# Adamtaranto/mimeo

Hardware: AMD Instinct MI355X
Metric: Gbp-aligned/sec (mimeo self, 1 Gbp genome, --minIdt 80 --minLen 100 --minCov 3) (higher is better)
Workload: dtype int32

## Files before the change

### mimeo_amd/csrc/device_util.h

```cpp
#pragma once
#include "common.h"

namespace mimeo {

#define MIMEO_AS_GLOBAL __attribute__((address_space(1)))
template <class T> struct gnative { using type = T; };
template <> struct gnative<uint2> { using type = uint32_t __attribute__((ext_vector_type(2))); };
template <> struct gnative<uint4> { using type = uint32_t __attribute__((ext_vector_type(4))); };
template <class T>
struct gptr {
    using N = typename gnative<T>::type;
    static_assert(sizeof(N) == sizeof(T), "the native twin has the layout of T");
    const MIMEO_AS_GLOBAL N *p;
    gptr() = default;
    __device__ __forceinline__ gptr(const T *q) : p((const MIMEO_AS_GLOBAL N *)q) {}
    __device__ __forceinline__ explicit gptr(const MIMEO_AS_GLOBAL N *q) : p(q) {}
    template <class I> __device__ __forceinline__ T operator[](I i) const { const N v = p[i]; return __builtin_bit_cast(T, v); }
    template <class I> __device__ __forceinline__ gptr operator+(I i) const { return gptr(p + i); }
    __device__ __forceinline__ explicit operator bool() const { return p != nullptr; }
    template <class U> __device__ __forceinline__ gptr<U> as() const { return gptr<U>((const MIMEO_AS_GLOBAL typename gnative<U>::type *)p); }
};
struct GStrandView {
    gptr<uint4> pw;
    gptr<uint32_t> svt;
// ... 37 lines not shown
    r.nm = (uint32_t)((((uint64_t)c.z << 32) | a.z) >> b);
    r.sv = (uint32_t)((((uint64_t)c.w << 32) | a.w) >> b);
    return r;
}
__device__ __forceinline__ Win64 win64(const GStrandView &v, int32_t s) {
    const int32_t w = s >> 5;
    const uint32_t b = (uint32_t)s & 31u;
    const uint4 a = v.pw[w], c = v.pw[w + 1], e = v.pw[w + 2];
    Win64 r;
    uint64_t l;
    l = ((uint64_t)c.x << 32) | a.x; r.lo = b ? (l >> b) | ((uint64_t)e.x << (64 - b)) : l;
    l = ((uint64_t)c.y << 32) | a.y; r.hi = b ? (l >> b) | ((uint64_t)e.y << (64 - b)) : l;
    l = ((uint64_t)c.z << 32) | a.z; r.nm = b ? (l >> b) | ((uint64_t)e.z << (64 - b)) : l;
    l = ((uint64_t)c.w << 32) | a.w; r.sv = b ? (l >> b) | ((uint64_t)e.w << (64 - b)) : l;
    return r;
}
template <class P>
__device__ __forceinline__ uint32_t get32(const P pl, int32_t s) {
    int32_t w = s >> 5;
    uint32_t b = (uint32_t)s & 31u;
    uint64_t v = (uint64_t)pl[w] | ((uint64_t)pl[w + 1] << 32);
    return (uint32_t)(v >> b);
}
__device__ __forceinline__ uint32_t seedvalid32(const GStrandView &v, int32_t s, uint32_t sv_from_window) {
    return v.svt ? get32(v.svt, s) : sv_from_window;
}
struct Base1 { uint32_t lo, hi, nm; };
__device__ __forceinline__ Base1 base_at(const GStrandView &v, int32_t s) {
    const uint4 a = v.pw[s >> 5];
    const uint32_t b = (uint32_t)s & 31u;
    return Base1{(a.x >> b) & 1u, (a.y >> b) & 1u, (a.z >> b) & 1u};
}

__device__ __forceinline__ int32_t sub_score(uint32_t dl, uint32_t dh, uint32_t cg, uint32_t nn) {
    uint32_t tb = dl ? 0x83858E8Eu : 0xE1E1645Bu;
    uint32_t sh = 24u - (((dh << 1) | cg) << 3);
    int32_t s = ((int32_t)(tb << sh)) >> 24;
    return nn ? -100 : s;
}

__device__ __forceinline__ int32_t pair_score(const GStrandView &T, const GStrandView &Q, int32_t pt, int32_t pq,
                                              bool *is_match) {
    const Base1 a = base_at(T, pt), b = base_at(Q, pq);
    const uint32_t dl = a.lo ^ b.lo, dh = a.hi ^ b.hi, nn = a.nm | b.nm;
    *is_match = !(dl | dh | nn);
    return sub_score(dl, dh, a.lo ^ a.hi, nn);
}

}
```

### mimeo_amd/csrc/k4_device.h

```cpp
#pragma once
#include "device_util.h"

namespace mimeo {

constexpr uint32_t CARE19 = 0x7A997u;
constexpr int EXT_THREADS = 256;
constexpr int LONG_WINDOWS = 8;

struct ExtCounters {
    unsigned long long ncand, nfollow, nlong, nhsp, nmed, nbig, nwalked;
    unsigned long long nfollow8[8], nmed8[8];
    unsigned long long nbigcand;
    unsigned long long long_next, seg_next;
    unsigned long long nwalk_total, nwalk_over;
    unsigned long long dbg[8];
};

struct HeavyPlan {
    const unsigned long long *est;
    uint2 *tile;
    uint32_t *base;
    uint4 *split;
    unsigned int *ctr;
};
struct Cand {
    uint32_t tstart, qstart, len;
    int32_t raw;
    uint32_t unit;
};
constexpr int32_t RAW_SATURATED = 0x7FFFFFFF;

struct ExtQueues {
    ExtCounters *ctr;
    Cand *cand;
    uint64_t *fkey;
    uint32_t *fprev;
    uint2 *medq, *longq;
    uint32_t *medu, *longu;
    uint2 *walkq;
    unsigned long long *nwalk_u;
    unsigned long long *nheavy_u;
    uint32_t *heavy;
    unsigned long long *heavy_est;
    unsigned long long *bigcand;
    unsigned long long *bigacc;
    unsigned long long *unit_hits;
    unsigned long long *tile_hits;
    uint64_t cand_cap, follow_cap, med_cap, long_cap, walk_cap;
    uint32_t ebits, dbits;
};
constexpr uint32_t WALK_SHARP_DONE = 0x80000000u;
__device__ __forceinline__ uint32_t queue_shard() { return blockIdx.x & 7u; }
__device__ __forceinline__ unsigned long long wave_slot(unsigned long long *counter) {
    const uint64_t m = __ballot(true);
    const uint32_t lane = threadIdx.x & 63u, lead = (uint32_t)__builtin_ctzll(m);
    unsigned long long b = 0;
    if (lane == lead) b = atomicAdd(counter, (unsigned long long)__popcll(m));
    b = __shfl(b, (int)lead);
    return b + __popcll(m & ((1ull << lane) - 1ull));
}
__device__ __forceinline__ uint64_t follow_key(const ExtQueues &q, uint32_t unit, int32_t d, uint32_t qlen, uint32_t et) {
    return ((uint64_t)unit << (q.dbits + q.ebits)) | ((uint64_t)(uint32_t)(d + (int32_t)qlen) << q.ebits) | (uint64_t)et;
}
__device__ __forceinline__ uint32_t key_unit(const ExtQueues &q, uint64_t k) { return (uint32_t)(k >> (q.dbits + q.ebits)); }
__device__ __forceinline__ uint32_t key_end(const ExtQueues &q, uint64_t k) { return (uint32_t)(k & ((1ull << q.ebits) - 1ull)); }
__device__ __forceinline__ uint64_t key_unit_diag(const ExtQueues &q, uint64_t k) { return k >> q.ebits; }
__device__ __forceinline__ int32_t key_diag(const ExtQueues &q, uint64_t k, uint32_t qlen) {
    return (int32_t)(uint32_t)((k >> q.ebits) & ((1ull << q.dbits) - 1ull)) - (int32_t)qlen;
}

// ... 87 lines not shown
    int32_t R = w.run, B = w.best, sR = R, sB = B;
    uint32_t BK = 0, sBK = 0, sC = 0;
    bool stopped = w.done, slow = false, brkdone = false;
#pragma unroll
    for (int c = 0; c < NG; c++) {
        const uint32_t e = ent[c];
        const int32_t S = ((int32_t)(e << 22)) >> 22, M = ((int32_t)(e << 12)) >> 22, mn = ((int32_t)(e << 2)) >> 22;
        const bool blk = (nz >> (G * c)) & 1u;
        const bool brk = R + mn + xdrop < B;
        const bool first = (blk || brk) && !stopped;
        sR = first ? R : sR;
        sB = first ? B : sB;
        sBK = first ? BK : sBK;
        sC = first ? (uint32_t)c : sC;
        slow = slow || (first && blk);
        brkdone = brkdone || (first && !blk);
        stopped = stopped || blk || brk;
        const int32_t cand = R + M;
        BK = cand > B ? (e >> 30) + (uint32_t)(G * c + 1) : BK;
        B = max(B, cand);
        R += S;
    }
    if (!stopped) { sR = R; sB = B; sBK = BK; sC = NG; }
    w.run = sR;
    w.best = sB;
    w.bk = sBK ? w.k + sBK : w.bk;
    w.k += (uint32_t)G * sC;
    w.done = w.done || brkdone;
    if (__ballot(slow)) {
        if (slow) walk_window<G>(tab, w, mdl, mdh, mcg, mnn, mH, limit, xdrop, (uint32_t)G * sC);
    }
}

template <int G>
__device__ __forceinline__ uint32_t group_table_entry(uint32_t idx) {
    int32_t p = 0, M = -100000, mn = 100000, posM = 0;
#pragma unroll
    for (int k = 0; k < G; k++) {
        p += sub_score((idx >> k) & 1u, (idx >> (G + k)) & 1u, (idx >> (2 * G + k)) & 1u, 0u);
        if (p > M) { M = p; posM = k; }
        if (p < mn) mn = p;
    }
    return ((uint32_t)p & 0x3FFu) | (((uint32_t)M & 0x3FFu) << 10) | (((uint32_t)mn & 0x3FFu) << 20) | ((uint32_t)posM << 30);
}

__device__ __forceinline__ uint32_t ext32(uint32_t a, uint32_t b, uint32_t c, uint32_t sh) {
    return sh < 32 ? __builtin_amdgcn_alignbit(b, a, sh) : __builtin_amdgcn_alignbit(c, b, sh - 32);
}

struct Frame {
    uint32_t dl[6], dh[6], cg[6], nn[6], st[6], sq[6];
};

struct WinMasks { uint32_t dl, dh, cg, nn, H; };

template <int WIN>
__device__ __forceinline__ WinMasks left_masks(const Frame &F, uint32_t bt, int transitions) {
    constexpr int b = 1 - WIN;
    const uint32_t dllo = __builtin_amdgcn_alignbit(F.dl[b + 1], F.dl[b], bt), dlhi = __builtin_amdgcn_alignbit(F.dl[b + 2], F.dl[b + 1], bt);
    const uint32_t dhlo = __builtin_amdgcn_alignbit(F.dh[b + 1], F.dh[b], bt), dhhi = __builtin_amdgcn_alignbit(F.dh[b + 2], F.dh[b + 1], bt);
    const uint32_t cglo = __builtin_amdgcn_alignbit(F.cg[b + 1], F.cg[b], bt), cghi = __builtin_amdgcn_alignbit(F.cg[b + 2], F.cg[b + 1], bt);
    const uint32_t nnlo = __builtin_amdgcn_alignbit(F.nn[b + 1], F.nn[b], bt), nnhi = __builtin_amdgcn_alignbit(F.nn[b + 2], F.nn[b + 1], bt);
    const uint32_t nlo = dllo | dhlo, nhi = dlhi | dhhi;
    uint32_t ones = 0, twos = 0, tv = 0;
#pragma unroll
    for (int c = 0; c < SEED_LEN; c++) {
// ... 120 lines not shown
            t2 |= __builtin_amdgcn_alignbit(dllo, dlm, c);
        }
        m.H2 = ~(transitions ? (w2 | t2) : o2) & 0xFFFF0000u;
    }
    return m;
}

template <int STEP, bool SLIM>
__device__ __forceinline__ bool hit_needs_walk(const GStrandView &T, const GStrandView &Q, const uint2 h, int xdrop,
                                               int hspthresh, int transitions) {
    Frame F;
    if (SLIM) load_frame_slim(T, Q, h, F);
    else load_frame(T, Q, h, F);
    const uint32_t bt = h.x & 31u;
    const FilterMasks l0 = filter_left<0>(F, bt, transitions), l1 = filter_left<1>(F, bt, transitions);
    const uint32_t rs = bt + SEED_LEN;
    Bound L{0, 0, 0, 0, false}, R{0, 0, 0, 0, false};
    bound_window<STEP, true>(L, l0.dl, l0.dh, l0.cg, xdrop);
    bound_window<STEP, true>(L, l1.dl, l1.dh, l1.cg, xdrop);
    const bool stop64 = L.stop;
    bound_window<16, true, 1>(L, l1.dl2, l1.dh2, l1.cg2, xdrop);
    const uint32_t veto2 = stop64 ? 0u : l1.H2;
    bound_window<STEP, false>(R, ext32(F.dl[2], F.dl[3], F.dl[4], rs), ext32(F.dh[2], F.dh[3], F.dh[4], rs),
                              ext32(F.cg[2], F.cg[3], F.cg[4], rs), xdrop);
    bound_window<STEP, false>(R, ext32(F.dl[3], F.dl[4], F.dl[5], rs), ext32(F.dh[3], F.dh[4], F.dh[5], rs),
                              ext32(F.cg[3], F.cg[4], F.cg[5], rs), xdrop);
    const uint32_t veto = F.nn[0] | F.nn[1] | F.nn[2] | F.nn[3] | F.nn[4] | F.nn[5] | l0.H | l1.H | veto2;
    return !(L.stop && R.stop && L.ub + R.ub < hspthresh && veto == 0);
}

template <int VARIANT>
__device__ __forceinline__ void walk_hit(const uint32_t *__restrict__ tab, const GStrandView &T, const GStrandView &Q,
                                         const uint2 h, int xdrop, int hspthresh, int transitions, bool &q_med,
                                         bool &q_fol, bool &q_cd, uint64_t &r_fk, uint32_t &r_fp, Cand &r_cd) {
    const int32_t et = (int32_t)h.x + SEED_LEN, eq = (int32_t)h.y + SEED_LEN;
    const int32_t d = (int32_t)h.x - (int32_t)h.y;
    const uint32_t bt = h.x & 31u;
    Frame F;
    if (VARIANT == 8) {
        const uint32_t bq = h.y & 31u;
        const int32_t wt = (int32_t)(h.x >> 5) - 2, wq = (int32_t)(h.y >> 5) - 2 - (bq < bt ? 1 : 0);
        const gptr<uint2> t2 = T.pw.as<uint2>(), q2 = Q.pw.as<uint2>();
        uint32_t acc = 0;
#pragma unroll
        for (int k = 0; k < 6; k++) { const uint2 v = t2[wt + k]; acc ^= v.x ^ v.y; }
#pragma unroll
        for (int k = 0; k < 7; k++) { const uint2 v = q2[wq + k]; acc ^= v.x ^ v.y; }
        if (acc == 0x12345678u) q_med = true;
        return;
    }
    if (VARIANT == 3) {
#pragma unroll
        for (int k = 0; k < 6; k++) {
            F.dl[k] = h.x * (k + 1); F.dh[k] = h.y + k; F.cg[k] = h.y * (k + 3); F.nn[k] = 0; F.st[k] = ~0u; F.sq[k] = ~0u;
        }
    } else {
        load_frame(T, Q, h, F);
    }
    if (VARIANT == 2) {
        uint32_t acc = 0;
#pragma unroll
        for (int k = 0; k < 6; k++) acc ^= F.dl[k] ^ F.dh[k] ^ F.cg[k] ^ F.nn[k] ^ F.st[k] ^ F.sq[k];
        if (acc == 0x12345678u) q_med = true;
        return;
    }
    WalkState L{0, 0, 0, 0, false, false, 0};
    const uint32_t maxl = (uint32_t)min(et, eq);
    left_window<0>(tab, F, bt, transitions, L, maxl, xdrop);
    if (!L.done) left_window<1>(tab, F, bt, transitions, L, maxl, xdrop);
    if (!L.done) {
        q_med = true;
    } else if (L.found) {
        q_fol = true;
        r_fk = ((uint64_t)(uint32_t)(d + (int32_t)Q.len) << 32) | (uint32_t)et;
        r_fp = (uint32_t)et - L.found_step;
        if (L.found_step == 1) {
            const bool two_back = seed_hit_at(T, Q, (int32_t)h.x - 2, d, transitions), ahead = seed_hit_at(T, Q, (int32_t)h.x + 1, d, transitions);
            if (two_back && ahead) q_fol = false;
            else if (two_back) r_fp = RUN_END;
        }
    } else {
        WalkState R{0, 0, 0, 0, false, false, 0};
        const uint32_t maxr = min(T.len - (uint32_t)et, Q.len - (uint32_t)eq);
        const uint32_t rs = bt + SEED_LEN;
        walk_window_pred(tab, R, ext32(F.dl[2], F.dl[3], F.dl[4], rs), ext32(F.dh[2], F.dh[3], F.dh[4], rs),
                         ext32(F.cg[2], F.cg[3], F.cg[4], rs), ext32(F.nn[2], F.nn[3], F.nn[4], rs), 0u, maxr, xdrop);
        if (!R.done)
            walk_window_pred(tab, R, ext32(F.dl[3], F.dl[4], F.dl[5], rs), ext32(F.dh[3], F.dh[4], F.dh[5], rs),
                             ext32(F.cg[3], F.cg[4], F.cg[5], rs), ext32(F.nn[3], F.nn[4], F.nn[5], rs), 0u, maxr, xdrop);
        if (!R.done) {
            q_med = true;
        } else if (L.best + R.best >= hspthresh) {
            q_cd = true;
            r_cd = Cand{(uint32_t)et - L.bk, (uint32_t)eq - L.bk, L.bk + R.bk, L.best + R.best, 0u};
        }
    }
}

struct WaveFill { uint32_t n_med, n_fol, n_cd; };

__device__ __forceinline__ uint64_t batch_key(const ExtQueues &q, uint32_t unit, uint64_t staged) {
    return ((uint64_t)unit << (q.dbits + q.ebits)) | ((staged >> 32) << q.ebits) | (staged & 0xFFFFFFFFull);
}

template <bool STAGE_CAND, int CAP = QCAP>
__device__ __forceinline__ void stage_records(const ExtQueues &q, uint32_t unit, uint2 *s_med, uint64_t *s_fk, uint32_t *s_fp,
                                              Cand *s_cd, WaveFill &f, bool q_med, uint2 h, bool q_fol, uint64_t r_fk,
                                              uint32_t r_fp, bool q_cd, Cand r_cd, bool final) {
    const uint32_t lane = threadIdx.x & 63u;
    const uint64_t lt_mask = (1ull << lane) - 1ull;
    uint64_t m = __ballot(q_med);
    if (m || (final && f.n_med)) {
        const uint32_t add = (uint32_t)__popcll(m);
        if (f.n_med + add > (uint32_t)CAP || (final && !m)) {
            __builtin_amdgcn_wave_barrier();
            unsigned long long b = 0;
            if (lane == 0) b = atomicAdd(&q.ctr->nmed8[queue_shard()], (unsigned long long)f.n_med);
            b = __shfl(b, 0);
            for (uint32_t i = lane; i < f.n_med; i += 64)
                if (b + i < q.med_cap) { const size_t at = (size_t)queue_shard() * q.med_cap + b + i; q.medq[at] = s_med[i]; q.medu[at] = unit; }
            f.n_med = 0;
            __builtin_amdgcn_wave_barrier();
        }
        if (q_med) s_med[f.n_med + __popcll(m & lt_mask)] = h;
        f.n_med += add;
        if (final && f.n_med) {
            __builtin_amdgcn_wave_barrier();
            unsigned long long b = 0;
            if (lane == 0) b = atomicAdd(&q.ctr->nmed8[queue_shard()], (unsigned long long)f.n_med);
            b = __shfl(b, 0);
            for (uint32_t i = lane; i < f.n_med; i += 64)
                if (b + i < q.med_cap) { const size_t at = (size_t)queue_shard() * q.med_cap + b + i; q.medq[at] = s_med[i]; q.medu[at] = unit; }
            f.n_med = 0;
        }
    }
    m = __ballot(q_fol);
    if (m || (final && f.n_fol)) {
        const uint32_t add = (uint32_t)__popcll(m);
        if (f.n_fol + add > (uint32_t)CAP || (final && !m)) {
            __builtin_amdgcn_wave_barrier();
            unsigned long long b = 0;
            if (lane == 0) b = atomicAdd(&q.ctr->nfollow8[queue_shard()], (unsigned long long)f.n_fol);
            b = __shfl(b, 0);
            for (uint32_t i = lane; i < f.n_fol; i += 64)
                if (b + i < q.follow_cap) { const size_t at = (size_t)queue_shard() * q.follow_cap + b + i; q.fkey[at] = batch_key(q, unit, s_fk[i]); q.fprev[at] = s_fp[i]; }
            f.n_fol = 0;
            __builtin_amdgcn_wave_barrier();
        }
        if (q_fol) { const uint32_t i = f.n_fol + __popcll(m & lt_mask); s_fk[i] = r_fk; s_fp[i] = r_fp; }
        f.n_fol += add;
        if (final && f.n_fol) {
            __builtin_amdgcn_wave_barrier();
            unsigned long long b = 0;
            if (lane == 0) b = atomicAdd(&q.ctr->nfollow8[queue_shard()], (unsigned long long)f.n_fol);
            b = __shfl(b, 0);
            for (uint32_t i = lane; i < f.n_fol; i += 64)
                if (b + i < q.follow_cap) { const size_t at = (size_t)queue_shard() * q.follow_cap + b + i; q.fkey[at] = batch_key(q, unit, s_fk[i]); q.fprev[at] = s_fp[i]; }
// ... 297 lines not shown
```

### mimeo_amd/csrc/k4_extend.hip

```cpp
#include <algorithm>
#include <cmath>
#include <cstdio>
#include <cstdlib>
#include <cstring>
#include <mutex>
#include <utility>

#include <rocprim/rocprim.hpp>

#include "k4_device.h"

namespace mimeo {

__global__ __launch_bounds__(EXT_THREADS) void k4_extend_generic(const UnitDesc *__restrict__ units, ExtQueues q, int xdrop,
                                                              int hspthresh, int transitions,
                                                              const uint32_t *__restrict__ group_tab) {
    __shared__ uint32_t tab[GROUP_TAB];
    for (int i = threadIdx.x; i < GROUP_TAB; i += EXT_THREADS) tab[i] = group_tab[i];
    __syncthreads();
    uint64_t sh_end[8];
    {
        uint64_t acc = 0;
#pragma unroll
        for (int r = 0; r < 8; r++) { acc += min((uint64_t)q.ctr->nmed8[r], q.med_cap); sh_end[r] = acc; }
// ... 18 lines not shown
        __builtin_amdgcn_wave_barrier();
    };
    auto flush_long = [&]() {
        __builtin_amdgcn_wave_barrier();
        unsigned long long b = 0;
        if (lane == 0) b = atomicAdd(&q.ctr->nlong, (unsigned long long)n_long);
        b = __shfl(b, 0) + lane;
        if (lane < n_long && b < q.long_cap) { q.longq[b] = s_lh[wv][lane]; q.longu[b] = s_lu[wv][lane]; }
        n_long = 0;
        __builtin_amdgcn_wave_barrier();
    };
    auto flush_cd = [&]() {
        __builtin_amdgcn_wave_barrier();
        unsigned long long b = 0;
        if (lane == 0) b = atomicAdd(&q.ctr->ncand, (unsigned long long)n_cd);
        b = __shfl(b, 0) + lane;
        if (lane < n_cd && b < q.cand_cap) q.cand[b] = s_cd[wv][lane];
        n_cd = 0;
        __builtin_amdgcn_wave_barrier();
    };
    const uint64_t stride = (uint64_t)gridDim.x * EXT_THREADS;
    for (uint64_t g0 = (uint64_t)blockIdx.x * EXT_THREADS + wv * 64u; g0 < nhits; g0 += stride) {
        const uint64_t gid = g0 + lane;
        bool o_fol = false, o_long = false, o_cd = false;
        uint64_t r_fk = 0;
        uint32_t r_fp = 0, unit = 0;
        uint2 h = make_uint2(0, 0);
        Cand r_cd{0, 0, 0, 0, 0};
        if (gid < nhits) {
            uint32_t r = 0;
#pragma unroll
            for (int k = 0; k < 7; k++) r += gid >= sh_end[k] ? 1u : 0u;
            const uint64_t at = (uint64_t)r * q.med_cap + (gid - (r ? sh_end[r - 1] : 0));
            h = q.medq[at];
            unit = q.medu[at];
            const GStrandView T = units[unit].T, Q = units[unit].Q;
            const int32_t et = (int32_t)h.x + SEED_LEN, eq = (int32_t)h.y + SEED_LEN;
            const int32_t d = (int32_t)h.x - (int32_t)h.y;
            WalkState L{0, 0, 0, 0, false, false, 0};
            const uint32_t maxl = (uint32_t)min(et, eq);
            bool is_long = false;
            for (int win = 0; !L.done; win++) {
                if (win == LONG_WINDOWS) { is_long = true; break; }
                const int32_t P = et - 32 * (win + 1) - SEED_LEN, Pq = P - d;
                const Win64 tw = win64(T, P), qw = win64(Q, Pq);
                const uint64_t dl64 = tw.lo ^ qw.lo, dh64 = tw.hi ^ qw.hi, nm64 = dl64 | dh64;
                const uint32_t nlo = (uint32_t)nm64, nhi = (uint32_t)(nm64 >> 32);
                const uint32_t tlo = (uint32_t)dl64, thi = (uint32_t)(dl64 >> 32);
                uint32_t ones = 0, twos = 0, tv = 0;
#pragma unroll
                for (int c = 0; c < SEED_LEN; c++) {
                    if (!((CARE19 >> c) & 1u)) continue;
                    const uint32_t v = c ? __builtin_amdgcn_alignbit(nhi, nlo, c) : nlo;
                    twos |= ones & v;
                    ones |= v;
                    tv |= c ? __builtin_amdgcn_alignbit(thi, tlo, c) : tlo;
                }
                const uint32_t bad = transitions ? (twos | tv) : ones;
                const uint32_t H = ~bad & seedvalid32(T, P, (uint32_t)tw.sv) & (uint32_t)qw.sv;
                walk_window(tab, L, __brev((uint32_t)(dl64 >> SEED_LEN)), __brev((uint32_t)(dh64 >> SEED_LEN)),
                            __brev((uint32_t)((tw.lo ^ tw.hi) >> SEED_LEN)), __brev((uint32_t)((tw.nm | qw.nm) >> SEED_LEN)),
                            __brev(H), maxl, xdrop);
            }
            if (!is_long && L.found) {
                o_fol = true;
                r_fk = follow_key(q, unit, d, Q.len, (uint32_t)et);
                r_fp = (uint32_t)et - L.found_step;
            } else {
                WalkState R{0, 0, 0, 0, false, false, 0};
                if (!is_long) {
                    const uint32_t maxr = min(T.len - (uint32_t)et, Q.len - (uint32_t)eq);
                    for (int win = 0; !R.done; win++) {
                        if (win == LONG_WINDOWS) { is_long = true; break; }
                        const int32_t P = et + 32 * win, Pq = P - d;
                        const Win32 tw = win32(T, P), qw = win32(Q, Pq);
                        walk_window(tab, R, tw.lo ^ qw.lo, tw.hi ^ qw.hi, tw.lo ^ tw.hi, tw.nm | qw.nm, 0u, maxr, xdrop);
                    }
                }
                if (is_long) o_long = true;
                else {
                    const int32_t score = L.best + R.best;
                    if (score >= hspthresh) { o_cd = true; r_cd = Cand{(uint32_t)et - L.bk, (uint32_t)eq - L.bk, L.bk + R.bk, score, unit}; }
                }
            }
        }
        uint64_t m = __ballot(o_fol);
        if (m) {
            const uint32_t add = (uint32_t)__popcll(m);
            if (n_fol + add > GCAP) flush_fol();
            if (o_fol) { const uint32_t i = n_fol + (uint32_t)__popcll(m & lt_mask); s_fk[wv][i] = r_fk; s_fp[wv][i] = r_fp; }
            n_fol += add;
        }
        m = __ballot(o_long);
        if (m) {
            const uint32_t add = (uint32_t)__popcll(m);
            if (n_long + add > GCAP) flush_long();
            if (o_long) { const uint32_t i = n_long + (uint32_t)__popcll(m & lt_mask); s_lh[wv][i] = h; s_lu[wv][i] = unit; }
            n_long += add;
        }
        m = __ballot(o_cd);
        if (m) {
            const uint32_t add = (uint32_t)__popcll(m);
            if (n_cd + add > GCAP) flush_cd();
            if (o_cd) s_cd[wv][n_cd + (uint32_t)__popcll(m & lt_mask)] = r_cd;
            n_cd += add;
        }
    }
    if (n_fol) flush_fol();
    if (n_long) flush_long();
    if (n_cd) flush_cd();
}

template <int VARIANT>
__device__ __forceinline__ void extend_hits_body(const GStrandView &T, const GStrandView &Q,
                                                 const uint2 *__restrict__ hits, uint64_t nhits,
                                                 int xdrop, int hspthresh, int transitions,
                                                 const uint32_t *__restrict__ group_tab, const ExtQueues &q, uint32_t unit,
                                                 int skip_diag0, const unsigned long long *__restrict__ nhits_dev) {
    constexpr bool FILTER = VARIANT == 5 || VARIANT == 9;
    constexpr int SCAP = 256;
    uint64_t sh_end[8] = {0, 0, 0, 0, 0, 0, 0, 0};
    const uint64_t shard_cap = nhits;
    if (nhits_dev) {
        uint64_t acc = 0;
#pragma unroll
        for (int r = 0; r < 8; r++) { acc += min((uint64_t)nhits_dev[r], shard_cap); sh_end[r] = acc; }
        nhits = acc;
    }
    __shared__ uint32_t tab[GROUP_TAB];
    __shared__ uint2 s_med[FAST_THREADS / 64][SCAP];
    __shared__ uint64_t s_fk[FAST_THREADS / 64][SCAP];
    __shared__ uint32_t s_fp[FAST_THREADS / 64][SCAP];
    __shared__ Cand s_cd[FAST_THREADS / 64][QCAP];
    __shared__ uint2 s_walk[FILTER ? FAST_THREADS / 64 : 1][QCAP];
    for (int i = threadIdx.x; i < GROUP_TAB; i += FAST_THREADS) tab[i] = group_tab[i];
    __syncthreads();
    const uint32_t lane = threadIdx.x & 63u, wv = threadIdx.x >> 6;
    const uint64_t lt_mask = (1ull << lane) - 1ull;
    WaveFill fill{0, 0, 0};
    uint32_t n_walk = 0, n_walked = 0;

    auto walk_batch = [&](bool active, uint2 h, bool final) {
        bool q_med = false, q_fol = false, q_cd = false;
        uint64_t r_fk = 0;
        uint32_t r_fp = 0;
        Cand r_cd{0, 0, 0, 0, 0};
        if (active) walk_hit<1>(tab, T, Q, h, xdrop, hspthresh, transitions, q_med, q_fol, q_cd, r_fk, r_fp, r_cd);
        stage_records<true, SCAP>(q, unit, s_med[wv], s_fk[wv], s_fp[wv], s_cd[wv], fill, q_med, h, q_fol, r_fk, r_fp, q_cd, r_cd, final);
    };

    const uint64_t stride = (uint64_t)gridDim.x * FAST_THREADS;
    for (uint64_t g0 = (uint64_t)blockIdx.x * FAST_THREADS + wv * 64u; g0 < nhits; g0 += stride) {
        const uint64_t gid = g0 + lane;
        uint2 h = make_uint2(0, 0);
        if (gid < nhits) {
            uint64_t at = gid;
            if (nhits_dev) {
                uint32_t r = 0;
#pragma unroll
                for (int k = 0; k < 7; k++) r += gid >= sh_end[k] ? 1u : 0u;
                at = (uint64_t)r * shard_cap + (gid - (r ? sh_end[r - 1] : 0));
            }
            h = hits[at];
        }
        const bool marked = nhits_dev && (h.x & WALK_SHARP_DONE) != 0;
        if (nhits_dev) h.x &= POS_MASK;
        const bool valid = gid < nhits && !(skip_diag0 && h.x == h.y);
        if (!FILTER) {
            walk_batch(valid, h, false);
        } else {
            bool need = valid && marked;
            if (__ballot(valid && !marked)) {
                if (valid && !marked)
                    need = VARIANT == 9 ? hit_needs_walk<16, true>(T, Q, h, xdrop, hspthresh, transitions)
                                        : hit_needs_walk<16, false>(T, Q, h, xdrop, hspthresh, transitions);
            }
            const uint64_t m = __ballot(need);
            if (m) {
                const uint32_t add = (uint32_t)__popcll(m);
                if (n_walk + add > (uint32_t)QCAP) {
                    __builtin_amdgcn_wave_barrier();
// ... 431 lines not shown
            out_unit[i] = c.unit;
        }
    }
}

__global__ __launch_bounds__(256) void k4_mirror_hsps(mimeo_hsp *__restrict__ hsps, uint32_t *__restrict__ hsp_unit, uint64_t nh,
                                                      const uint32_t *__restrict__ mirror_dst, unsigned long long *__restrict__ ctr) {
    for (uint64_t i = (uint64_t)blockIdx.x * 256 + threadIdx.x; i < nh; i += (uint64_t)gridDim.x * 256) {
        const uint32_t m = mirror_dst[hsp_unit[i]];
        if (m == NO_MIRROR) continue;
        const unsigned long long at = nh + wave_slot(ctr);
        mimeo_hsp h = hsps[i];
        const uint32_t t = h.tstart;
        h.tstart = h.qstart; h.qstart = t;
        hsps[at] = h;
        hsp_unit[at] = m;
    }
}

static uint32_t *g_group_tab = nullptr;
static std::once_flag g_group_once;

const uint32_t *group_table_device() {
    std::call_once(g_group_once, [&] {
        std::vector<uint32_t> tab(GROUP_TAB);
        build_group_table(tab.data());
        if (hipMalloc((void **)&g_group_tab, GROUP_TAB * 4) != hipSuccess ||
            hipMemcpy(g_group_tab, tab.data(), GROUP_TAB * 4, hipMemcpyHostToDevice) != hipSuccess)
            g_group_tab = nullptr;
    });
    return g_group_tab;
}

int launch_fused_batch(const FusedUnit *d_units, uint32_t nactive, const ExtQueues &q, const HeavyPlan &plan, const mimeo_params *p, hipStream_t st,
                       uint32_t dbg);
void launch_sum_hits(const ExtQueues &q, uint32_t nunits, hipStream_t st);

void ExtBatch::release() {
    for (DeviceBuf *b : {&units, &ctr, &cand, &fkey, &fkey2, &fprev, &fprev2, &medq, &medu, &longq, &longu, &walkq, &flags, &segs, &tmp,
                         &nsel, &bigseg, &hsps, &hsp_unit, &unit_hits, &tile_hits, &selfs, &hits, &bigcand, &bigacc, &heavy, &mirror, &funits, &nwalk_u, &plan_buf, &arena_q, &arena_s})
        b->release();
    jc.release();
    for (auto &e : ev) { if (e) (void)hipEventDestroy(e); e = nullptr; }
    for (auto &e : kev) (void)hipEventDestroy(e);
    kev.clear();
    if (side_done) { (void)hipEventDestroy(side_done); side_done = nullptr; }
    if (side) { (void)hipStreamDestroy(side); side = nullptr; }
    delete (ExtQueues *)q_;
    q_ = nullptr;
    started_ = false;
}

static uint32_t bits_for(uint64_t v) {
    uint32_t b = 1;
    while (b < 64 && (v >> b)) b++;
    return b;
}

uint32_t ext_batch_max_units(uint64_t max_tlen, uint64_t max_qlen) {
    const uint32_t ebits = bits_for(max_tlen + SEED_LEN), dbits = bits_for(max_tlen + max_qlen + SEED_LEN);
    const uint32_t ubits = 64 - std::min(63u, ebits + dbits);
    return ubits >= 20 ? (1u << 20) : (1u << ubits);
}

int ExtBatch::run(const std::vector<UnitWork> &work, const mimeo_params *p, uint64_t *nhsp_out, ExtStats *stats,
                  const std::vector<uint32_t> *mirror_dst) {
    *nhsp_out = 0;
    if (work.empty()) return 0;
    int rc = start(work, p, mirror_dst);
    if (rc) return rc;
    return finish(nhsp_out, stats);
}

uint64_t ExtBatch::arena_bytes() const {
    const uint64_t mf = mirror_dst_.empty() ? 1 : 2;
    return cap_f_ * 8 * 12 + cap_m_ * 8 * 12 + cap_l_ * 12 + cap_c_ * (sizeof(Cand) + mf * (sizeof(mimeo_hsp) + 4)) + (v1_ ? 8 : walk_entries_ * 8) + 4096;
}
uint64_t ExtBatch::queue_bytes() const {
    const uint64_t mf = mirror_dst_.empty() ? 1 : 2;
    return arena_bytes() + cap_f_ * 8 * 41 + cap_c_ * mf * 260;
}
static void *carve(const DeviceBuf &arena, size_t *off, size_t bytes) {
    void *p = (char *)arena.p + *off;
    *off += (bytes + 255) & ~(size_t)255;
    return p;
}
void ExtBatch::release_queues() {
    for (DeviceBuf *d : {&cand, &fkey, &fkey2, &fprev, &fprev2, &medq, &medu, &longq, &longu, &walkq, &flags, &segs, &tmp, &bigseg, &hsps, &hsp_unit})
        d->release();
    arena_q.release();
    arena_s.release();
}
uint64_t ExtBatch::held_bytes() const { return arena_q.cap + arena_s.cap; }
static int queue_budget(const ExtBatch &b, uint64_t *budget) {
    size_t free_b = 0, total_b = 0;
    HIP_TRY(hipMemGetInfo(&free_b, &total_b));
    const uint64_t have = (uint64_t)free_b + b.held_bytes(), reserve = std::min<uint64_t>(have / 8, 8ull << 30);
    *budget = have - reserve;
    if (getenv("MIMEO_QUEUE_BUDGET_MB")) *budget = (uint64_t)atol(getenv("MIMEO_QUEUE_BUDGET_MB")) << 20;
    return 0;
}

int ExtBatch::start(const std::vector<UnitWork> &work, const mimeo_params *p, const std::vector<uint32_t> *mirror_dst) {
    hipStream_t st = stream();
    started_ = false;
    const uint32_t nunits = (uint32_t)work.size();
    if (!nunits) return 0;
    w_ = work;
    p_ = *p;
// ... 68 lines not shown
        if (getenv("MIMEO_TRACE"))
            fprintf(stderr, "[trace] batch of %u units, %.3g expected hits: queues %.2f GiB of %.2f GiB budget (boosts f %.1f m %.1f l %.1f c %.1f w %.1f; caps f %llu m %llu l %llu c %llu walk entries %llu)\n", nunits, expect_hits,
                    (double)queue_bytes() / (1 << 30), (double)budget / (1 << 30), boost_f, boost_m, boost_l, boost_c, boost_w,
                    (unsigned long long)cap_f_, (unsigned long long)cap_m_, (unsigned long long)cap_l_, (unsigned long long)cap_c_, (unsigned long long)walk_entries_);
        if (splittable_ && queue_bytes() > budget) return MIMEO_ERR_SPLIT;
    }
    if (!mirror_dst_.empty()) {
        if ((rc = mirror.reserve((size_t)nunits * 4 + 16))) return rc;
        HIP_TRY(hipMemcpyAsync(mirror.p, mirror_dst_.data(), (size_t)nunits * 4, hipMemcpyHostToDevice, st));
    }
    if (!q_) q_ = new ExtQueues();
    if ((rc = enqueue_heavy())) return rc;
    started_ = true;
    return 0;
}

int ExtBatch::enqueue_heavy() {
    hipStream_t st = stream();
    const uint32_t nunits = (uint32_t)w_.size();
    const mimeo_params *p = &p_;
    const uint32_t *tab = group_table_device();
    if (!tab) { set_error("group table upload failed"); return MIMEO_ERR_HIP; }
    ExtQueues &q = *(ExtQueues *)q_;
    memset(&q, 0, sizeof q);
    q.ebits = ebits_; q.dbits = dbits_;
    const uint64_t cap_f = cap_f_, cap_m = cap_m_, cap_l = cap_l_, cap_c = cap_c_;
    const bool v1 = v1_;
    const std::vector<UnitWork> &work = w_;
    const std::vector<uint32_t> &h_selfs = h_selfs_;
    int rc;
    {
        {
            const size_t mf = mirror_dst_.empty() ? 1 : 2;
            const size_t sz[10] = {cap_f * 8 * 8, cap_f * 8 * 4, cap_m * 8 * 8, cap_m * 8 * 4, cap_l * 8, cap_l * 4, cap_c * sizeof(Cand),
                                   cap_c * sizeof(mimeo_hsp) * mf, cap_c * 4 * mf, v1 ? 8 : walk_entries_ * 8 + 8};
            size_t total = 0;
            for (size_t z : sz) total += (z + 255) & ~(size_t)255;
            if (total > arena_q.cap) {
                for (DeviceBuf *d : {&fkey, &fprev, &medq, &medu, &longq, &longu, &cand, &hsps, &hsp_unit, &walkq}) d->release();
                size_t free_b = 0, total_b = 0;
                HIP_TRY(hipMemGetInfo(&free_b, &total_b));
                const size_t have = free_b + arena_q.cap;
                size_t want = arena_q.cap ? total + total / 2 : total;
                if (want + (queue_bytes() - arena_bytes()) + (8ull << 30) > have) want = total;
                if ((rc = arena_q.reserve(want)) && want > total) rc = arena_q.reserve(total);
                if (rc) return rc == MIMEO_ERR_NOMEM && splittable_ ? MIMEO_ERR_SPLIT : rc;
            }
            size_t off = 0;
            DeviceBuf *bufs[10] = {&fkey, &fprev, &medq, &medu, &longq, &longu, &cand, &hsps, &hsp_unit, &walkq};
            for (int i = 0; i < 10; i++) bufs[i]->set_view(carve(arena_q, &off, sz[i]), sz[i]);
        }
        q.ctr = (ExtCounters *)ctr.p;
        q.cand = (Cand *)cand.p; q.fkey = (uint64_t *)fkey.p; q.fprev = (uint32_t *)fprev.p;
        q.medq = (uint2 *)medq.p; q.medu = (uint32_t *)medu.p; q.longq = (uint2 *)longq.p; q.longu = (uint32_t *)longu.p;
        q.bigcand = (unsigned long long *)bigcand.p; q.bigacc = (unsigned long long *)bigacc.p;
        q.unit_hits = (unsigned long long *)unit_hits.p;
        q.tile_hits = (unsigned long long *)tile_hits.p;
        q.walkq = (uint2 *)walkq.p;
        q.cand_cap = cap_c; q.follow_cap = cap_f; q.med_cap = cap_m; q.long_cap = cap_l; q.walk_cap = 0;
        const UnitDesc *d_units = (const UnitDesc *)units.p;
        HIP_TRY(hipMemsetAsync(ctr.p, 0, sizeof(ExtCounters), st));
        HIP_TRY(hipMemsetAsync(unit_hits.p, 0, (size_t)nunits * 8, st));
        if (!v1) HIP_TRY(hipMemsetAsync(tile_hits.p, 0, (size_t)nunits * NTILE * 8, st));
        HIP_TRY(hipMemsetAsync(nsel.p, 0, 16, st));
        HIP_TRY(hipMemsetAsync(bigacc.p, 0, (size_t)ENT_BIGCAP * 5 * 8, st));
        HIP_TRY(hipEventRecord(ev[0], st));
        if (!h_selfs.empty()) {
            HIP_TRY(hipStreamWaitEvent(side, ev[0], 0));
            hipLaunchKernelGGL(k4_diag0, dim3((uint32_t)h_selfs.size()), dim3(64), 0, side, d_units, (const uint32_t *)selfs.p, q,
                               p->xdrop, p->hspthresh, p->transitions);
            HIP_TRY(hipEventRecord(side_done, side));
        }
        if (!v1) {
            std::vector<FusedUnit> h_fu;
            bool slim = true;
            uint64_t base = 0;
            for (uint32_t u = 0; u < nunits; u++) {
                const UnitWork &w = work[u];
                if (!w.ti.n || !w.qi.n) continue;
                FusedUnit f;
                memset(&f, 0, sizeof f);
                f.T = w.ti; f.Q = w.qi; f.Tv = w.d.T; f.Qv = w.d.Q; f.unit = u; f.same = w.d.same;
                f.walk_base = base; f.walk_cap = walk_cap_u_[u];
                base += 8 * f.walk_cap;
                slim = slim && !w.d.T.has_n && !w.d.Q.has_n;
                h_fu.push_back(f);
            }
// ... 56 lines not shown
#undef K4_LAUNCH
            }
        }
        if (!v1) launch_sum_hits(q, nunits, st);
        HIP_TRY(hipEventRecord(ev[1], st));
    }
    HIP_TRY(hipGetLastError());
    return 0;
}

int ExtBatch::finish(uint64_t *nhsp_out, ExtStats *stats) {
    *nhsp_out = 0;
    if (!started_) return 0;
    started_ = false;
    hipStream_t st = stream();
    const uint32_t nunits = (uint32_t)w_.size();
    const mimeo_params *p = &p_;
    const uint32_t *tab = group_table_device();
    ExtQueues &q = *(ExtQueues *)q_;
    const std::vector<UnitWork> &work = w_;
    const std::vector<uint32_t> &h_selfs = h_selfs_;
    const bool v1 = v1_;
    const uint32_t key_bits = key_bits_;
    const double expect_hits = expect_hits_;
    const UnitDesc *d_units = (const UnitDesc *)units.p;
    int rc;
    ExtCounters c;
    uint64_t nf_total = 0, nm_total = 0;
    float ms_heavy = 0, ms_tails = 0, ms_walk = 0, ms_k34 = 0;
    for (int attempt = 0;; attempt++) {
        uint64_t &cap_f = cap_f_, &cap_m = cap_m_, &cap_l = cap_l_, &cap_c = cap_c_;
        HIP_TRY(hipStreamWaitEvent(st, ev[1], 0));
        HIP_TRY(hipEventRecord(ev[3], st));
        hipLaunchKernelGGL(k4_extend_generic, dim3(1024), dim3(EXT_THREADS), 0, st, d_units, q, p->xdrop, p->hspthresh,
                           p->transitions, tab);
        if (!h_selfs.empty()) HIP_TRY(hipStreamWaitEvent(st, side_done, 0));
        hipLaunchKernelGGL(k4_extend_long, dim3(768), dim3(EXT_THREADS), 0, st, d_units, q, p->xdrop, p->hspthresh, p->transitions);
        HIP_TRY(hipMemcpyAsync(&c, ctr.p, sizeof c, hipMemcpyDeviceToHost, st));
        HIP_TRY(hipStreamSynchronize(st));
        uint64_t nf = 0, nm = 0, maxf = 0, maxm = 0;
        for (int r = 0; r < 8; r++) {
            nf += std::min<uint64_t>(c.nfollow8[r], cap_f);
            nm += std::min<uint64_t>(c.nmed8[r], cap_m);
            maxf = std::max<uint64_t>(maxf, c.nfollow8[r]);
            maxm = std::max<uint64_t>(maxm, c.nmed8[r]);
        }
        nf_total = nf; nm_total = nm;
        bool over = maxf > cap_f || maxm > cap_m || c.nlong > cap_l || c.ncand > cap_c || c.nwalk_over > 1024;
        if (!over && nf) {
            size_t t1 = 0, t2 = 0;
            rocprim::counting_iterator<uint64_t> iota(0);
            HIP_TRY(rocprim::radix_sort_pairs(nullptr, t1, (uint64_t *)nullptr, (uint64_t *)nullptr, (uint32_t *)nullptr, (uint32_t *)nullptr, (size_t)nf, 0, key_bits, st));
            HIP_TRY(rocprim::select(nullptr, t2, iota, (uint8_t *)nullptr, (uint64_t *)nullptr, (uint64_t *)nsel.p, (size_t)nf, st));
            const size_t sz[6] = {nf * 8, nf * 4, nf, nf * 8, nf * 8, std::max(t1, t2) + 16};
            size_t total = 0;
            for (size_t z : sz) total += (z + 255) & ~(size_t)255;
            if (total > arena_s.cap) {
                for (DeviceBuf *d : {&fkey2, &fprev2, &flags, &segs, &bigseg, &tmp}) d->release();
                size_t free_b = 0, total_b = 0;
                HIP_TRY(hipMemGetInfo(&free_b, &total_b));
                size_t want = arena_s.cap ? total + total / 2 : total + total / 8;
                if (want + (4ull << 30) > free_b + arena_s.cap) want = total;
                if ((rc = arena_s.reserve(want)) && want > total) rc = arena_s.reserve(total);
                if (rc) return rc == MIMEO_ERR_NOMEM && splittable_ ? MIMEO_ERR_SPLIT : rc;
            }
            size_t off = 0;
            DeviceBuf *bufs[6] = {&fkey2, &fprev2, &flags, &segs, &bigseg, &tmp};
// ... 128 lines not shown
```

Baseline: 0.04560.

## Carry packed walk state in medium queue so generic extension resumes mid-walk

Medium-queue records grow from 8 to 16 bytes and now carry a packed snapshot of the x-drop walk state (run, best, best position, and the left result when the right side overflowed). The generic extension kernel resumes from that frame instead of re-walking the first FRAME_STEPS bases on each side, saving redundant scoring and window loads. In exchange it doubles medium-queue memory traffic and arena size, shrinks the shared staging buffer to 128 entries (more frequent flushes), and adds a trap if the walk depth differs from FRAME_STEPS. The generic kernel grid is also sized from occupancy times CU count instead of a fixed 1024.

```diff
diff --git a/mimeo_amd/csrc/device_util.h b/mimeo_amd/csrc/device_util.h
--- a/mimeo_amd/csrc/device_util.h
+++ b/mimeo_amd/csrc/device_util.h
@@ -93,12 +93,24 @@
     return Base1{(a.x >> b) & 1u, (a.y >> b) & 1u, (a.z >> b) & 1u};
 }
 
+constexpr uint32_t SUB_DL1 = 0x83858E8Eu, SUB_DL0 = 0xE1E1645Bu;
+constexpr int32_t SUB_N = -100;
 __device__ __forceinline__ int32_t sub_score(uint32_t dl, uint32_t dh, uint32_t cg, uint32_t nn) {
-    uint32_t tb = dl ? 0x83858E8Eu : 0xE1E1645Bu;
+    uint32_t tb = dl ? SUB_DL1 : SUB_DL0;
     uint32_t sh = 24u - (((dh << 1) | cg) << 3);
     int32_t s = ((int32_t)(tb << sh)) >> 24;
-    return nn ? -100 : s;
+    return nn ? SUB_N : s;
 }
+constexpr int32_t sub_extreme(bool largest) {
+    int32_t e = SUB_N;
+    for (int k = 0; k < 8; k++) {
+        const int32_t b = (int32_t)(((k < 4 ? SUB_DL0 : SUB_DL1) >> (8 * (k & 3))) & 0xFFu), s = b >= 128 ? b - 256 : b;
+        e = largest ? (s > e ? s : e) : (s < e ? s : e);
+    }
+    return e;
+}
+constexpr int32_t SUB_MAX = sub_extreme(true), SUB_MIN = sub_extreme(false);
+static_assert(SUB_MAX == 100 && SUB_MIN == -125, "HOXD70");
 
 __device__ __forceinline__ int32_t pair_score(const GStrandView &T, const GStrandView &Q, int32_t pt, int32_t pq,
                                               bool *is_match) {
diff --git a/mimeo_amd/csrc/k4_device.h b/mimeo_amd/csrc/k4_device.h
--- a/mimeo_amd/csrc/k4_device.h
+++ b/mimeo_amd/csrc/k4_device.h
@@ -35,7 +35,8 @@
     Cand *cand;
     uint64_t *fkey;
     uint32_t *fprev;
-    uint2 *medq, *longq;
+    uint4 *medq;
+    uint2 *longq;
     uint32_t *medu, *longu;
     uint2 *walkq;
     unsigned long long *nwalk_u;
@@ -189,6 +190,30 @@
     }
 }
 
+constexpr uint32_t FRAME_STEPS = 64;
+static_assert(-(int32_t)FRAME_STEPS * SUB_MIN < (1 << 13) && (int32_t)FRAME_STEPS * SUB_MAX < (1 << 13), "run: 14 bits signed, best: 13 bits");
+static_assert(FRAME_STEPS < (1u << 7), "bk: 7 bits");
+struct Resume {
+    uint32_t kind;
+    int32_t run, best;
+    uint32_t bk;
+    int32_t lbest;
+    uint32_t lbk;
+};
+__device__ __forceinline__ uint2 pack_resume(uint32_t kind, int32_t run, int32_t best, uint32_t bk, int32_t lbest, uint32_t lbk) {
+    return make_uint2(((uint32_t)run & 0x3FFFu) | ((uint32_t)best << 14) | (kind << 31), bk | (lbk << 7) | ((uint32_t)lbest << 14));
+}
+__device__ __forceinline__ Resume unpack_resume(uint32_t x, uint32_t y) {
+    Resume r;
+    r.kind = x >> 31;
+    r.run = ((int32_t)(x << 18)) >> 18;
+    r.best = (int32_t)((x >> 14) & 0x1FFFu);
+    r.bk = y & 0x7Fu;
+    r.lbk = (y >> 7) & 0x7Fu;
+    r.lbest = (int32_t)((y >> 14) & 0x1FFFu);
+    return r;
+}
+
 template <int G>
 __device__ __forceinline__ uint32_t group_table_entry(uint32_t idx) {
     int32_t p = 0, M = -100000, mn = 100000, posM = 0;
@@ -375,7 +400,7 @@
 template <int VARIANT>
 __device__ __forceinline__ void walk_hit(const uint32_t *__restrict__ tab, const GStrandView &T, const GStrandView &Q,
                                          const uint2 h, int xdrop, int hspthresh, int transitions, bool &q_med,
-                                         bool &q_fol, bool &q_cd, uint64_t &r_fk, uint32_t &r_fp, Cand &r_cd) {
+                                         uint2 &r_st, bool &q_fol, bool &q_cd, uint64_t &r_fk, uint32_t &r_fp, Cand &r_cd) {
     const int32_t et = (int32_t)h.x + SEED_LEN, eq = (int32_t)h.y + SEED_LEN;
     const int32_t d = (int32_t)h.x - (int32_t)h.y;
     const uint32_t bt = h.x & 31u;
@@ -412,7 +437,9 @@
     left_window<0>(tab, F, bt, transitions, L, maxl, xdrop);
     if (!L.done) left_window<1>(tab, F, bt, transitions, L, maxl, xdrop);
     if (!L.done) {
+        if (L.k != FRAME_STEPS) __builtin_trap();
         q_med = true;
+        r_st = pack_resume(0u, L.run, L.best, L.bk, 0, 0u);
     } else if (L.found) {
         q_fol = true;
         r_fk = ((uint64_t)(uint32_t)(d + (int32_t)Q.len) << 32) | (uint32_t)et;
@@ -432,7 +459,9 @@
             walk_window_pred(tab, R, ext32(F.dl[3], F.dl[4], F.dl[5], rs), ext32(F.dh[3], F.dh[4], F.dh[5], rs),
                              ext32(F.cg[3], F.cg[4], F.cg[5], rs), ext32(F.nn[3], F.nn[4], F.nn[5], rs), 0u, maxr, xdrop);
         if (!R.done) {
+            if (R.k != FRAME_STEPS) __builtin_trap();
             q_med = true;
+            r_st = pack_resume(1u, R.run, R.best, R.bk, L.best, L.bk);
         } else if (L.best + R.best >= hspthresh) {
             q_cd = true;
             r_cd = Cand{(uint32_t)et - L.bk, (uint32_t)eq - L.bk, L.bk + R.bk, L.best + R.best, 0u};
@@ -446,16 +475,17 @@
     return ((uint64_t)unit << (q.dbits + q.ebits)) | ((staged >> 32) << q.ebits) | (staged & 0xFFFFFFFFull);
 }
 
-template <bool STAGE_CAND, int CAP = QCAP>
-__device__ __forceinline__ void stage_records(const ExtQueues &q, uint32_t unit, uint2 *s_med, uint64_t *s_fk, uint32_t *s_fp,
-                                              Cand *s_cd, WaveFill &f, bool q_med, uint2 h, bool q_fol, uint64_t r_fk,
+template <bool STAGE_CAND, int CAP = QCAP, int MCAP = CAP>
+__device__ __forceinline__ void stage_records(const ExtQueues &q, uint32_t unit, uint4 *s_med, uint64_t *s_fk, uint32_t *s_fp,
+                                              Cand *s_cd, WaveFill &f, bool q_med, uint2 h, uint2 r_st, bool q_fol, uint64_t r_fk,
                                               uint32_t r_fp, bool q_cd, Cand r_cd, bool final) {
+    static_assert(MCAP >= 64 && CAP >= 64, "a batch adds up to 64 records of a kind");
     const uint32_t lane = threadIdx.x & 63u;
     const uint64_t lt_mask = (1ull << lane) - 1ull;
     uint64_t m = __ballot(q_med);
     if (m || (final && f.n_med)) {
         const uint32_t add = (uint32_t)__popcll(m);
-        if (f.n_med + add > (uint32_t)CAP || (final && !m)) {
+        if (f.n_med + add > (uint32_t)MCAP || (final && !m)) {
             __builtin_amdgcn_wave_barrier();
             unsigned long long b = 0;
             if (lane == 0) b = atomicAdd(&q.ctr->nmed8[queue_shard()], (unsigned long long)f.n_med);
@@ -465,7 +495,7 @@
             f.n_med = 0;
             __builtin_amdgcn_wave_barrier();
         }
-        if (q_med) s_med[f.n_med + __popcll(m & lt_mask)] = h;
+        if (q_med) s_med[f.n_med + __popcll(m & lt_mask)] = make_uint4(h.x, h.y, r_st.x, r_st.y);
         f.n_med += add;
         if (final && f.n_med) {
             __builtin_amdgcn_wave_barrier();
diff --git a/mimeo_amd/csrc/k4_extend.hip b/mimeo_amd/csrc/k4_extend.hip
--- a/mimeo_amd/csrc/k4_extend.hip
+++ b/mimeo_amd/csrc/k4_extend.hip
@@ -74,15 +74,18 @@
 #pragma unroll
             for (int k = 0; k < 7; k++) r += gid >= sh_end[k] ? 1u : 0u;
             const uint64_t at = (uint64_t)r * q.med_cap + (gid - (r ? sh_end[r - 1] : 0));
-            h = q.medq[at];
+            const uint4 rec = q.medq[at];
+            h = make_uint2(rec.x, rec.y);
             unit = q.medu[at];
+            const Resume rs = unpack_resume(rec.z, rec.w);
             const GStrandView T = units[unit].T, Q = units[unit].Q;
             const int32_t et = (int32_t)h.x + SEED_LEN, eq = (int32_t)h.y + SEED_LEN;
             const int32_t d = (int32_t)h.x - (int32_t)h.y;
-            WalkState L{0, 0, 0, 0, false, false, 0};
+            constexpr int RESUME_WIN = (int)(FRAME_STEPS / 32);
+            WalkState L{rs.kind ? 0 : rs.run, rs.kind ? rs.lbest : rs.best, rs.kind ? rs.lbk : rs.bk, rs.kind ? 0u : FRAME_STEPS, rs.kind != 0, false, 0};
             const uint32_t maxl = (uint32_t)min(et, eq);
             bool is_long = false;
-            for (int win = 0; !L.done; win++) {
+            for (int win = RESUME_WIN; !L.done; win++) {
                 if (win == LONG_WINDOWS) { is_long = true; break; }
                 const int32_t P = et - 32 * (win + 1) - SEED_LEN, Pq = P - d;
                 const Win64 tw = win64(T, P), qw = win64(Q, Pq);
@@ -109,10 +112,10 @@
                 r_fk = follow_key(q, unit, d, Q.len, (uint32_t)et);
                 r_fp = (uint32_t)et - L.found_step;
             } else {
-                WalkState R{0, 0, 0, 0, false, false, 0};
+                WalkState R{rs.kind ? rs.run : 0, rs.kind ? rs.best : 0, rs.kind ? rs.bk : 0u, rs.kind ? FRAME_STEPS : 0u, false, false, 0};
                 if (!is_long) {
                     const uint32_t maxr = min(T.len - (uint32_t)et, Q.len - (uint32_t)eq);
-                    for (int win = 0; !R.done; win++) {
+                    for (int win = rs.kind ? RESUME_WIN : 0; !R.done; win++) {
                         if (win == LONG_WINDOWS) { is_long = true; break; }
                         const int32_t P = et + 32 * win, Pq = P - d;
                         const Win32 tw = win32(T, P), qw = win32(Q, Pq);
@@ -161,6 +164,7 @@
                                                  int skip_diag0, const unsigned long long *__restrict__ nhits_dev) {
     constexpr bool FILTER = VARIANT == 5 || VARIANT == 9;
     constexpr int SCAP = 256;
+    constexpr int MCAP = 128;
     uint64_t sh_end[8] = {0, 0, 0, 0, 0, 0, 0, 0};
     const uint64_t shard_cap = nhits;
     if (nhits_dev) {
@@ -170,7 +174,7 @@
         nhits = acc;
     }
     __shared__ uint32_t tab[GROUP_TAB];
-    __shared__ uint2 s_med[FAST_THREADS / 64][SCAP];
+    __shared__ uint4 s_med[FAST_THREADS / 64][MCAP];
     __shared__ uint64_t s_fk[FAST_THREADS / 64][SCAP];
     __shared__ uint32_t s_fp[FAST_THREADS / 64][SCAP];
     __shared__ Cand s_cd[FAST_THREADS / 64][QCAP];
@@ -187,8 +191,9 @@
         uint64_t r_fk = 0;
         uint32_t r_fp = 0;
         Cand r_cd{0, 0, 0, 0, 0};
-        if (active) walk_hit<1>(tab, T, Q, h, xdrop, hspthresh, transitions, q_med, q_fol, q_cd, r_fk, r_fp, r_cd);
-        stage_records<true, SCAP>(q, unit, s_med[wv], s_fk[wv], s_fp[wv], s_cd[wv], fill, q_med, h, q_fol, r_fk, r_fp, q_cd, r_cd, final);
+        uint2 r_st = make_uint2(0, 0);
+        if (active) walk_hit<1>(tab, T, Q, h, xdrop, hspthresh, transitions, q_med, r_st, q_fol, q_cd, r_fk, r_fp, r_cd);
+        stage_records<true, SCAP, MCAP>(q, unit, s_med[wv], s_fk[wv], s_fp[wv], s_cd[wv], fill, q_med, h, r_st, q_fol, r_fk, r_fp, q_cd, r_cd, final);
     };
 
     const uint64_t stride = (uint64_t)gridDim.x * FAST_THREADS;
@@ -686,6 +691,23 @@
     return g_group_tab;
 }
 
+static uint32_t g_generic_grid = 0;
+static std::once_flag g_generic_once;
+static uint32_t generic_grid() {
+    std::call_once(g_generic_once, [&] {
+        int dev = 0, cus = 0, per_cu = 0;
+        if (hipGetDevice(&dev) == hipSuccess && hipDeviceGetAttribute(&cus, hipDeviceAttributeMultiprocessorCount, dev) == hipSuccess &&
+            hipOccupancyMaxActiveBlocksPerMultiprocessor(&per_cu, k4_extend_generic, EXT_THREADS, 0) == hipSuccess && cus > 0 && per_cu > 0)
+            g_generic_grid = (uint32_t)cus * (uint32_t)per_cu;
+        else {
+            g_generic_grid = 1024;
+            (void)hipGetLastError();
+        }
+        if (getenv("MIMEO_K4_STATS")) fprintf(stderr, "[k4] k4_extend_generic: %u workgroups (%d CUs x %d)\n", g_generic_grid, cus, per_cu);
+    });
+    return g_generic_grid;
+}
+
 int launch_fused_batch(const FusedUnit *d_units, uint32_t nactive, const ExtQueues &q, const HeavyPlan &plan, const mimeo_params *p, hipStream_t st,
                        uint32_t dbg);
 void launch_sum_hits(const ExtQueues &q, uint32_t nunits, hipStream_t st);
@@ -728,7 +750,7 @@
 
 uint64_t ExtBatch::arena_bytes() const {
     const uint64_t mf = mirror_dst_.empty() ? 1 : 2;
-    return cap_f_ * 8 * 12 + cap_m_ * 8 * 12 + cap_l_ * 12 + cap_c_ * (sizeof(Cand) + mf * (sizeof(mimeo_hsp) + 4)) + (v1_ ? 8 : walk_entries_ * 8) + 4096;
+    return cap_f_ * 8 * 12 + cap_m_ * 8 * 20 + cap_l_ * 12 + cap_c_ * (sizeof(Cand) + mf * (sizeof(mimeo_hsp) + 4)) + (v1_ ? 8 : walk_entries_ * 8) + 4096;
 }
 uint64_t ExtBatch::queue_bytes() const {
     const uint64_t mf = mirror_dst_.empty() ? 1 : 2;
@@ -863,7 +885,7 @@
     {
         {
             const size_t mf = mirror_dst_.empty() ? 1 : 2;
-            const size_t sz[10] = {cap_f * 8 * 8, cap_f * 8 * 4, cap_m * 8 * 8, cap_m * 8 * 4, cap_l * 8, cap_l * 4, cap_c * sizeof(Cand),
+            const size_t sz[10] = {cap_f * 8 * 8, cap_f * 8 * 4, cap_m * 8 * 16, cap_m * 8 * 4, cap_l * 8, cap_l * 4, cap_c * sizeof(Cand),
                                    cap_c * sizeof(mimeo_hsp) * mf, cap_c * 4 * mf, v1 ? 8 : walk_entries_ * 8 + 8};
             size_t total = 0;
             for (size_t z : sz) total += (z + 255) & ~(size_t)255;
@@ -883,7 +905,7 @@
         }
         q.ctr = (ExtCounters *)ctr.p;
         q.cand = (Cand *)cand.p; q.fkey = (uint64_t *)fkey.p; q.fprev = (uint32_t *)fprev.p;
-        q.medq = (uint2 *)medq.p; q.medu = (uint32_t *)medu.p; q.longq = (uint2 *)longq.p; q.longu = (uint32_t *)longu.p;
+        q.medq = (uint4 *)medq.p; q.medu = (uint32_t *)medu.p; q.longq = (uint2 *)longq.p; q.longu = (uint32_t *)longu.p;
         q.bigcand = (unsigned long long *)bigcand.p; q.bigacc = (unsigned long long *)bigacc.p;
         q.unit_hits = (unsigned long long *)unit_hits.p;
         q.tile_hits = (unsigned long long *)tile_hits.p;
@@ -1006,7 +1028,7 @@
         uint64_t &cap_f = cap_f_, &cap_m = cap_m_, &cap_l = cap_l_, &cap_c = cap_c_;
         HIP_TRY(hipStreamWaitEvent(st, ev[1], 0));
         HIP_TRY(hipEventRecord(ev[3], st));
-        hipLaunchKernelGGL(k4_extend_generic, dim3(1024), dim3(EXT_THREADS), 0, st, d_units, q, p->xdrop, p->hspthresh,
+        hipLaunchKernelGGL(k4_extend_generic, dim3(generic_grid()), dim3(EXT_THREADS), 0, st, d_units, q, p->xdrop, p->hspthresh,
                            p->transitions, tab);
         if (!h_selfs.empty()) HIP_TRY(hipStreamWaitEvent(st, side_done, 0));
         hipLaunchKernelGGL(k4_extend_long, dim3(768), dim3(EXT_THREADS), 0, st, d_units, q, p->xdrop, p->hspthresh, p->transitions);
```

Result: faster. 0.04619 (median of 6 runs) (+1.3%).
